# Emieeel/auto_oo

Measured on AMD Instinct MI355X. Metric: OO-VQE energy+grad evals/sec (formaldimine CAS(4e,3o)/cc-pVDZ); 2e-transform fp64 TFLOP/s vs roofline, higher is better.
Workload: dtype f64; 1 GPU; configs[1] shape: N=43 AOs, n_occ=6, CAS(4e,3o), UCCD n_theta=4, n_kappa=327; one step = one batched call evaluating energy + full gradient of all 256 geometries of the rank (256 synthetic geometries in the job, geometry g on rank g mod n_gpus); value = evaluations/s; in-order calls on one stream; geometries_per_rank=256, batched_calls=1332, calls=in order, parallelism=geometry-sharded x1, one all_gather at the end, dist_world_size=1, devices_visible=1, device_of_rank0=0

## Files before the change

### auto_oo_amd/csrc/cas.hip

```cpp
#include "plan.h"
#include "circuit_small.h"
#include <type_traits>
#include <stdlib.h>

namespace {

constexpr int HALF_WAVES = 8;
constexpr int TRI_REG_R = 3;
constexpr int tiles_depth(int zt) { return zt == 3 ? 4 : 8; }
constexpr int stream_depth(int zt) { return zt == 3 ? 2 : 3; }
constexpr int AUX_PLAIN = 0, AUX_NT = 2;

constexpr int SYM_FULL = 0, SYM_MIRROR = 1, SYM_PACKED = 2;
__device__ __forceinline__ void tri_decode(long t, int N, int& p, int& q)
{
    const double b = 2.0 * N + 1.0;
    int pp = (int)((b - sqrt(b * b - 8.0 * (double)t)) * 0.5);
    pp = pp < 0 ? 0 : (pp > N - 1 ? N - 1 : pp);
    while (pp > 0 && (long)pp * (2 * N - pp + 1) / 2 > t) --pp;
    while (pp < N - 1 && (long)(pp + 1) * (2 * N - pp) / 2 <= t) ++pp;
    p = pp;
    q = pp + (int)(t - (long)pp * (2 * N - pp + 1) / 2);
}

// ... 2354 lines not shown
            const long idx = base + u * 512 + tid;
            if (idx < (long)nrdm * n_kappa) gvec[idx] = 2.0 * (frc[u] - fcr[u]);
        }
    }
    if (fock)
        for (int idx = tid; idx < N * N; idx += 512) {
            const int m = idx / N;
            fock[idx] = m < M ? Fcol[idx] : 0.0;
        }
    if (gmat)
        for (int idx = tid; idx < N * N; idx += 512) {
            const int m = idx / N, n = idx - m * N;
            const double fmn = m < M ? Fcol[(size_t)m * N + n] : 0.0;
            const double fnm = n < M ? Fcol[(size_t)n * N + m] : 0.0;
            gmat[idx] = 2.0 * (fmn - fnm);
        }
    if (tid < nrdm) {
        const int k = tid;
        double acc = 0.0;
        for (int n = 0; n < M; ++n) acc += Epart[(size_t)k * N + n];
        if (k == 0) {
            double core = nuc;
            for (int n = 0; n < M; ++n) core += Cpart[n];
            c0[0] = core;
            E[0] = core + acc;
        } else if (dE) {
            dE[k - 1] = acc;
        }
    }
}

constexpr int TAIL_THREADS = 512;

__host__ __device__ inline bool tail_needed(int x, int y, int z, int no)
{
    const int lo = y < z ? y : z, hi = y < z ? z : y;
    if (lo >= no) return true;
    if (hi < no) return lo == hi || x == lo || x == hi;
    return x >= no || x == lo;
}
__host__ __device__ inline int tail_pitch(int NC) { return 16 * (((NC + 15) / 16) | 1); }

#ifdef OOVQE_TAIL_PROBE
constexpr int TAIL_PROBE_WGS = 512, TAIL_PROBE_MARKS = 32;
__device__ long long g_tail_probe[TAIL_PROBE_WGS][TAIL_PROBE_MARKS];
#define TAIL_MARK(i)                                                                              \
    do {                                                                                          \
        __syncthreads();                                                                          \
        if (threadIdx.x == 0 && blockIdx.x < TAIL_PROBE_WGS && (i) < TAIL_PROBE_MARKS)            \
            g_tail_probe[blockIdx.x][i] = wall_clock64();                                         \
    } while (0)
#else
#define TAIL_MARK(i) do {} while (0)
#endif

template <int KS>
__global__ __launch_bounds__(TAIL_THREADS, 2)
void cas_tail_kernel(const double* __restrict__ J, const double* __restrict__ C, const double* __restrict__ Wpre,
                     const double* __restrict__ gamma, const double* __restrict__ Gamma, int nrdm, int N, int no,
                     int na, int NC, double nuc, const double* __restrict__ nuc_arr,
                     const int32_t* __restrict__ kap_row, const int32_t* __restrict__ kap_col, int n_kappa,
                     double* __restrict__ c0, double* __restrict__ E, double* __restrict__ gvec,
                     double* __restrict__ dE, double* __restrict__ c1, double* __restrict__ c2, size_t out_stride)
{
    extern __shared__ double lds[];
    constexpr int NW = TAIL_THREADS / 64;
    constexpr int PW = (4 * KS + NW - 1) / NW;
    constexpr int GR = 2, NG = (PW + GR - 1) / GR;
    constexpr int NTN = (4 * KS + 15) / 16;
    const int M = no + na, M2 = M * M, M3 = M2 * M;
    const int na2 = na * na, na3 = na2 * na, na4 = na2 * na2;
    const int ncol = M * (M + 1) / 2, nty = (ncol + 15) / 16;
    const long tri = (long)N * (N + 1) / 2;
    const int by = blockIdx.x;
    const int tid = threadIdx.x, lane = tid & 63;
    const int wave = __builtin_amdgcn_readfirstlane(tid >> 6);
    const int lq = lane >> 4, lr = lane & 15;
    {
        const size_t gi = by;
        J += gi * nty * tri * 16;
        C += gi * (size_t)N * N;
        Wpre += gi * (size_t)N * N;
        gamma += gi * (size_t)nrdm * na2;
        Gamma += gi * (size_t)nrdm * na4;
        c0 += gi * out_stride;
        E += gi * out_stride;
        gvec += gi * out_stride;
        if (dE) dE += gi * out_stride;
        c1 += gi * out_stride;
        c2 += gi * out_stride;
        if (nuc_arr) nuc = nuc_arr[gi];
    }
    const int LDG = tail_pitch(NC), nct = (NC + 15) / 16;
    double* Gc = lds;
    double* Cl = Gc + (size_t)4 * KS * LDG;
    double* hn = Cl + (size_t)N * M;
// ... 47 lines not shown
        }
    };
    auto mfma_group = [&](const double (&af)[KS], const double (&bf)[GR][KS], const int (&tj)[4], int g) {
#pragma unroll
        for (int r = 0; r < GR; ++r) {
            const int i = g * GR + r;
            if (i >= PW) continue;
            int wv = wave;
#if defined(__HIP_DEVICE_COMPILE__)
            asm volatile("" : "+s"(wv));
#endif
            const int p = wv + NW * i;
            if (p >= 4 * KS) continue;
            d4 acc = d4{0.0, 0.0, 0.0, 0.0};
            if (p < N) {
#pragma unroll
                for (int ks = 0; ks < KS; ++ks) acc = mfma_f64(af[ks], bf[r][ks], acc);
            }
            double* row = Gc + p * LDG;
#pragma unroll
            for (int j = 0; j < 4; ++j)
                if (tj[j] >= 0) row[tj[j]] = acc[j];
        }
    };
    double bs[2][GR][KS];
    TAIL_MARK(0);
#pragma unroll
    for (int s0 = 0; s0 < 2; ++s0) load_group(bs[s0], s0 / NG, s0 % NG);

    for (int idx = tid; idx < N * M; idx += TAIL_THREADS) {
        const int q = idx / M, x = idx - q * M;
        Cl[idx] = C[(size_t)q * N + x];
    }
    for (int idx = tid; idx < N * N; idx += TAIL_THREADS) scr[idx] = Wpre[idx];
    for (int idx = tid; idx < nrdm * na2; idx += TAIL_THREADS) gml[idx] = gamma[idx];
    for (int idx = tid; idx < nrdm * na4; idx += TAIL_THREADS) Gml[idx] = Gamma[idx];
    for (int idx = tid; idx < n_kappa; idx += TAIL_THREADS) {
        krow[idx] = kap_row[idx];
        kcol[idx] = kap_col[idx];
    }
    for (int idx = tid; idx < 4 * KS * (LDG - NC); idx += TAIL_THREADS) {
        const int p = idx / (LDG - NC);
        Gc[p * LDG + NC + (idx - p * (LDG - NC))] = 0.0;
    }
    TAIL_MARK(1);
    {
        const int total = M * ncol;
        int base = 0;
        for (int i0 = 0; i0 < total; i0 += TAIL_THREADS) {
            const int i = i0 + tid;
            int x = 0, y = 0, z = 0;
            bool need = false;
            if (i < total) {
                x = i / ncol;
                tri_decode(i - x * ncol, M, y, z);
                need = tail_needed(x, y, z, no);
            }
            const unsigned long long mask = __ballot(need);
            const int below = __popcll(mask & ((1ull << lane) - 1ull));
            if (lane == 0) wcnt[wave] = __popcll(mask);
            __syncthreads();
            int pre = base, all = 0;
            for (int w = 0; w < NW; ++w) {
                const int c = wcnt[w];
                if (w < wave) pre += c;
                all += c;
            }
            if (i < total) {
                const int v = need ? pre + below : -1;
                tab[(x * M + y) * M + z] = v;
                tab[(x * M + z) * M + y] = v;
                tabp[i] = v;
            }
            __syncthreads();
            base += all;
        }
    }
    TAIL_MARK(2);
    for (int idx = tid; idx < N * M; idx += TAIL_THREADS) {
        const int n = idx / M, x = idx - n * M;
        double acc = 0.0;
        for (int q = 0; q < N; ++q) acc += scr[(size_t)n * N + q] * Cl[q * M + x];
        hn[idx] = acc;
    }
    __syncthreads();
    TAIL_MARK(3);

    {
        double af[KS];
#pragma unroll
        for (int ks = 0; ks < KS; ++ks) {
            const int q = 4 * ks + lq;
            const double c = Cl[(q < N ? q : N - 1) * M + (lr < M ? lr : 0)];
            af[ks] = (q < N && lr < M) ? c : 0.0;
        }
        auto tail_tile = [&](auto par, int ty) {
            constexpr int P = decltype(par)::value;
            const int yz = 16 * ty + lr;
            int tj[4];
#pragma unroll
            for (int j = 0; j < 4; ++j) {
                const int x = lq + 4 * j;
                tj[j] = (x < M && yz < ncol) ? tabp[x * ncol + yz] : -1;
            }
#pragma unroll
            for (int g = 0; g < NG; ++g) {
                mfma_group(af, bs[(P + g) & 1], tj, g);
                __builtin_amdgcn_sched_barrier(0);
                load_group(bs[(P + g) & 1], ty + (g + 2) / NG, (g + 2) % NG);
                __builtin_amdgcn_sched_barrier(0);
            }
        };
// ... 463 lines not shown

static size_t tail_lds_bytes(int N, int no, int na, int nrdm, int n_kappa, int* NC)
{
    const int M = no + na, M3 = M * M * M;
    Stage1Variant v;
    if (N > 48 || M > 16 || stage1_variant(N, &v)) return 0;
    int nc = 0;
    for (int x = 0; x < M; ++x)
        for (int y = 0; y < M; ++y)
            for (int z = y; z < M; ++z) nc += tail_needed(x, y, z, no) ? 1 : 0;
    *NC = nc;
    const size_t na2 = (size_t)na * na, na4 = na2 * na2;
    size_t scr = (size_t)N * N + ((size_t)M * (M * (M + 1) / 2) + 1) / 2;
    const size_t gc = (size_t)4 * tail_depth(N, v) * tail_pitch(nc);
    const size_t fe = (size_t)nrdm * M * N + (size_t)nrdm * N +
                      (size_t)N * na * na * na + (size_t)N * no * na2;
    if (fe > scr) scr = fe;
    const size_t doubles = gc + 3 * (size_t)N * M + (size_t)nrdm * (na2 + na4) + N +
                           ((size_t)M3 + TAIL_THREADS / 64 + 2 * (size_t)n_kappa + 1) / 2 + scr;
    const size_t bytes = doubles * sizeof(double);
    return bytes <= 160 * 1024 ? bytes : 0;
}

static int cas_tail_batched(const CasEvalArgs& a, const EvalPlan& p, const double* J, const double* Wpre, hipStream_t st)
{
    Stage1Variant v;
    if (int rc = stage1_variant(a.N, &v)) return rc;
#define OOVQE_LAUNCH_TAIL(KS_)                                                                    \
    do {                                                                                          \
        if (int rc_ = oovqe_ensure_dynamic_lds((const void*)cas_tail_kernel<KS_>, p.tail_lds)) return rc_; \
        hipLaunchKernelGGL((cas_tail_kernel<KS_>), dim3(a.batch), dim3(TAIL_THREADS), p.tail_lds, st, J, a.C, Wpre, \
                           a.gamma, a.Gamma, a.nrdm, a.N, a.n_occ, a.ncas, p.tail_nc, a.nuc, a.nuc_arr, a.kap_row, \
                           a.kap_col, a.n_kappa, a.out.c0, a.out.E, a.out.gvec, a.out.dE, a.out.c1, a.out.c2,       \
                           a.out_stride);                                                         \
    } while (0)
    oovqe_profile_mark_start_l(st, LABEL_P_TO_N);
    OOVQE_TAIL_DISPATCH(tail_depth(a.N, v), OOVQE_LAUNCH_TAIL)
    oovqe_profile_mark_stop(st);
#undef OOVQE_LAUNCH_TAIL
    OOVQE_CHECK_LAUNCH("cas_eval/tail");
    return 0;
}

static bool fused_plan(int N, int M, int batch, int n_cu, long chunks_opt, FusedPlan* fp)
{
    if (M > 16 || N > 48 || N < 1) return false;
    const long m2 = (long)M * M, m3 = m2 * M;
    if (chunks_opt <= 0 && (long)batch * N * N < 48L * n_cu) return false;
    long target = n_cu / batch;
    long nchunk0 = chunks_opt > 0 ? chunks_opt : target / N;
    if (nchunk0 < 1) nchunk0 = 1;
    const long cap = (2L * N * m2 - m3) / (m3 + N);
    if (cap < 1) return false;
    if (nchunk0 > cap) nchunk0 = cap;
    int qc = N, nchunk = 1;
    if (nchunk0 > 1) {
        qc = 4 * (int)((N + 4 * nchunk0 - 1) / (4 * nchunk0));
        nchunk = (N + qc - 1) / qc;
    }
    const int QR = (qc + 3) & ~3, CR = (nchunk - 1) * qc + QR;
    int ldb = (int)((m2 + 15) / 16 * 16);
    if (ldb % 32 == 0) ldb += 16;
    const size_t fixed = ((size_t)CR * 16 + 64 + 8) * sizeof(double);
    const size_t block = (size_t)QR * ldb * sizeof(double);
    const size_t task_stage = (size_t)m3 * sizeof(double);
    const long Tg = (long)nchunk * N;
    long wpg = target < 1 ? 1 : target;
// ... 290 lines not shown
                  "cas_eval: bad sizes");
    OOVQE_REQUIRE(s.batch >= 1 && s.batch <= 65535, "cas_eval: batch=%d", s.batch);
    OOVQE_REQUIRE(s.n_cu >= 1, "cas_eval: n_cu=%d", s.n_cu);
    const EvalOpts& o = s.opt;
    const int N = s.N, M = s.n_occ + s.ncas, batch = s.batch, nrdm = s.nrdm;
    const long m2 = (long)M * M, m3 = m2 * M;
    const long tri = (long)N * (N + 1) / 2;
    const long nty16 = (m2 + 15) / 16 * 16;
    const bool pq = (s.eri_flags & OOVQE_ERI_PQ_SYMMETRIC) != 0;
    p.rs = (s.eri_flags & OOVQE_ERI_RS_SYMMETRIC) != 0 && !o.sym_no_rs;

    const bool fused = !o.cas_unfused && fused_plan(N, M, batch, s.n_cu, o.fused_chunks, &p.fused);
    const bool packed = fused && pq && !o.sym_mirror && tri * nty16 + 2 * (long)N * m3 <= 2 * (long)N * N * m2;
    const bool two_step = o.sym_simple || o.sym_two_step;

    if (s.n_qubits > 0) {
        p.circuit = CIRCUIT_OWN;
        p.circuit_small = oovqe_circuit_rdms_is_small(s.n_qubits, s.ncas, nrdm, s.n_gates) != 0;
        if (p.circuit_small && o.no_ride != 1) {
            const long K = fused ? (long)p.fused.nchunk * N : N, B = fused ? m3 : (long)N * m2;
            bool ride = oovqe_small_circuit_lds_bytes(s.n_qubits, s.ncas, nrdm, s.n_gates) <= 64 * 1024 &&
                        K <= 0x7fffffffL && oovqe_contract_hosts_circuit(1, (int)K, N, B, 0, batch, o.k1);
            if (ride && fused && pq && !o.sym_mirror && o.no_ride != 2) {
                const long ntile = ((p.rs ? (long)M * (M + 1) / 2 : m2) + 15) / 16;
                if ((ntile + 1) * batch > 3L * s.n_cu) ride = false;
            }
            if (ride) p.circuit = CIRCUIT_RIDES;
        }
    }
    p.w = packed && !two_step && !o.panel_no_w && p.circuit == CIRCUIT_OWN && p.circuit_small && batch <= 32767;
    if (p.w && p.rs && s.packed && !s.t2_ready && !s.extras && 2L * batch > (long)s.n_cu && !o.tail_split)
        p.tail_lds = tail_lds_bytes(N, s.n_occ, s.ncas, nrdm, s.n_kappa, &p.tail_nc);
    if (p.tail_lds == 0 && N > m3) p.w = false;
    if (packed)
        p.path = p.tail_lds > 0 ? PATH_PACKED_TAIL : two_step ? PATH_PACKED_TWO_STEP : PATH_PACKED_SPLIT;
    else if (fused)
        p.path = PATH_FUSED;
    else
        p.path = column_fits(N, M, s.ncas) ? PATH_COLUMN : PATH_STAGED;
    OOVQE_REQUIRE(p.path != PATH_STAGED || M < N,
                  "cas_eval: the staged path needs at least one virtual orbital (N=%d M=%d)", N, M);
    if (p.path == PATH_STAGED && p.circuit == CIRCUIT_RIDES) p.circuit = CIRCUIT_OWN;

    Stage1Variant v;
    if (packed || fused)
        if (int rc = stage1_variant(N, &v)) return rc;
    if (!packed && fused) {
        p.stage1 = stage1_small(S1_FUSED, v, 0);
    } else if (!packed) {
        if (int rc = stage1_half(N, M, pq ? SYM_MIRROR : SYM_FULL, p.rs, N > 48 && s.packed, &p.stage1)) return rc;
    } else if (o.sym_simple) {
        if (int rc = stage1_half(N, M, SYM_PACKED, false, false, &p.stage1)) return rc;
    } else if (s.t2_ready && !two_step) {
        p.stage1.kernel = S1_FROM_T2;
    } else {
        p.stage1 = stage1_small(!two_step && p.rs && s.packed ? S1_TRI_REG : S1_TRI, v, two_step ? 0 : p.rs ? 2 : 1);
    }

    const size_t nb = (size_t)batch;
    size_t at = 0;
    auto block = [&](WorkBlock b, size_t doubles) { p.off[b] = at; p.len[b] = nb * doubles; at += nb * doubles; };
    if (packed) {
        block(WB_JP, (size_t)(tri * nty16));
        block(WB_T3, (size_t)N * m3);
        block(WB_GMW, (size_t)N * m3);
        if (!two_step) p.len[WB_T3] = p.w ? nb * N * N : 0;
// ... 356 lines not shown
    hipStream_t st = (hipStream_t)a.cas.stream;

    CasEvalArgs c = a.cas;
    c.gamma = a.work;
    c.Gamma = c.gamma + nb * nvec * na2;
    c.nrdm = nvec;
    c.work = a.work + nb * nvec * (na2 + na4);
    c.out = out_layout(a.out, nvec, c.n_kappa, c.ncas);
    c.out_stride = (size_t)oovqe_oo_eval_out_size(a.n_theta, c.n_kappa, c.ncas, a.derivatives);

    EvalPlan p;
    if (int rc = oovqe_eval_plan(eval_shape(c, a.n_qubits, a.n_gates), &p)) return rc;

    oovqe_circuit_job_t cj;
    if (p.circuit == CIRCUIT_RIDES) {
        cj = oovqe_circuit_job_t{.theta = a.theta, .gates = a.gates, .gamma = const_cast<double*>(c.gamma),
                                 .Gamma = const_cast<double*>(c.Gamma), .n_theta = a.n_theta, .n_gates = a.n_gates,
                                 .n_qubits = a.n_qubits, .ncas = a.cas.ncas, .n_tan = nvec - 1, .count = a.cas.batch,
                                 .init_index = a.init_index,
                                 .lds_bytes = oovqe_small_circuit_lds_bytes(a.n_qubits, a.cas.ncas, nvec, a.n_gates)};
        c.cj = &cj;
    } else {
        double *psi = nullptr, *dpsi = nullptr, *rwork = nullptr;
        if (!p.circuit_small) {
            psi = c.work + nb * oovqe_cas_eval_work_size(a.cas.N, a.cas.n_occ, a.cas.ncas, nvec);
            dpsi = psi + nb * D;
            rwork = psi + nb * nvec * D;
        }
        oovqe_profile_mark_start_l(st, LABEL_CIRCUIT);
        int rc = oovqe_circuit_rdms_w(a.theta, a.n_theta, a.gates, a.n_gates, a.n_qubits, a.cas.ncas, a.init_index,
                                      a.derivatives, a.cas.batch, psi, a.derivatives ? dpsi : nullptr,
                                      const_cast<double*>(c.gamma), const_cast<double*>(c.Gamma), rwork,
                                      p.w ? a.cas.h_ao : nullptr, p.w ? a.cas.C : nullptr, a.cas.N,
                                      p.w ? c.work + p.off[WB_T3] : nullptr, a.cas.stream);
        if (rc) return rc;
        oovqe_profile_mark_stop(st);
        if (c.rdm_event) {
            OOVQE_CHECK_HIP(hipEventRecord(c.rdm_event, st), "oo_eval: hipEventRecord");
            c.rdm_event = nullptr;
        }
    }
    return cas_eval_batched(c, p);
}

int oovqe_half_transform_batched_impl(const double* g_ao, const double* C, int N, int M, double* T2,
                                      int batch, unsigned eri_flags, oovqe_stream_t stream, double* Vk_tri)
{
    const bool pq = (eri_flags & OOVQE_ERI_PQ_SYMMETRIC) != 0;
    const bool rs = (eri_flags & OOVQE_ERI_RS_SYMMETRIC) != 0 && oovqe_opt(OOVQE_OPT_SYM_NO_RS) == 0;
    Stage1 s;
    if (int rc = stage1_half(N, M, pq ? SYM_MIRROR : SYM_FULL, rs, false, &s)) return rc;
    return half_transform_batched(g_ao, C, N, M, T2, batch, stream, s, Vk_tri);
}

extern "C" int oovqe_oo_eval_batch(const double* theta, int n_theta, const oovqe_gate_t* gates,
                                   int n_gates, int n_qubits, uint32_t init_index, const double* g_ao,
                                   const double* h_ao, const double* C, const double* nuc, int N,
                                   int n_occ, int ncas, const int32_t* kap_row, const int32_t* kap_col,
                                   int n_kappa, int derivatives, int batch, double* work, double* out,
                                   unsigned eri_flags, const double* g_packed, oovqe_stream_t stream)
{
    OOVQE_REQUIRE(nuc, "oo_eval_batch: null nuc");
    return oovqe_oo_eval_batched_impl(OoEvalArgs{
        .theta = theta, .n_theta = n_theta, .gates = gates, .n_gates = n_gates, .n_qubits = n_qubits,
        .init_index = init_index, .derivatives = derivatives, .work = work, .out = out,
        .cas = {.g_ao = g_ao, .h_ao = h_ao, .C = C, .nuc_arr = nuc, .N = N, .n_occ = n_occ, .ncas = ncas,
                .kap_row = kap_row, .kap_col = kap_col, .n_kappa = n_kappa, .batch = batch, .stream = stream,
// ... 21 lines not shown
{
    static thread_local char line[1024];
    static const char* const path_names[] = {"packed_tail", "packed_split", "packed_two_step", "fused", "column", "staged"};
    static const char* const circuit_names[] = {"none", "rides", "own"};
    static const char* const block_names[WB_COUNT] = {"Jp", "T3", "Gmw", "Cdup", "T2", "U", "Fcol", "Epart", "Cpart"};
    const EvalShape s{.N = N, .n_occ = n_occ, .ncas = ncas, .nrdm = derivatives ? 1 + n_theta : 1, .n_kappa = n_kappa,
                      .batch = batch, .eri_flags = eri_flags, .packed = have_packed != 0, .n_qubits = n_qubits,
                      .n_gates = n_gates, .n_cu = oovqe_cu_count(), .opt = oovqe_eval_opts()};
    EvalPlan p;
    if (n_qubits != 0 && n_qubits != 2 * ncas) {
        oovqe_set_error("oo_eval: n_qubits != 2*ncas");
        return nullptr;
    }
    if (oovqe_eval_plan(s, &p)) return nullptr;
    const bool k1 = p.path == PATH_PACKED_TWO_STEP || p.path == PATH_FUSED || p.path == PATH_COLUMN;
    const long M = n_occ + ncas, K = p.path == PATH_FUSED ? (long)p.fused.nchunk * N : N;
    const int hosts = k1 && oovqe_contract_hosts_circuit(1, (int)K, N, p.path == PATH_COLUMN ? N * M * M : M * M * M, 0, batch, s.opt.k1);
    size_t n = 0;
    auto add = [&](const char* fmt, auto... args) {
        if (n < sizeof(line)) n += (size_t)snprintf(line + n, sizeof(line) - n, fmt, args...);
    };
    add("path=%s; stage1=%s; circuit=%s; w=%d; launches=%ld; k1_hosts=%d; labels=", path_names[p.path], p.stage1.name,
        circuit_names[p.circuit], p.w ? 1 : 0, p.launches, hosts);
    for (int l = 0; l < LABEL_COUNT; ++l) add("%s%d", l ? "," : "", p.labels[l]);
    add("%s", "; blocks=");
    for (int b = 0, first = 1; b < WB_COUNT; ++b)
        if (p.len[b]) {
            add("%s%s@%zu+%zu", first ? "" : ",", block_names[b], p.off[b], p.len[b]);
            first = 0;
        }
    if (p.path == PATH_PACKED_TAIL) {
        Stage1Variant v;
        if (stage1_variant(N, &v)) return nullptr;
        add("; tail=cas_tail_kernel<%d>; tail_lds=%zu", tail_depth(N, v), p.tail_lds);
    }
    if (p.path == PATH_FUSED)
        add("; nchunk=%d; qc=%d; nbuf=%d; wpg=%d", p.fused.nchunk, p.fused.qc, p.fused.nbuf, p.fused.wpg);
    if (p.path == PATH_PACKED_SPLIT || p.path == PATH_PACKED_TWO_STEP || p.path == PATH_FUSED) {
        PanelGeom pg;
        const bool panel_w = p.w && p.path == PATH_PACKED_SPLIT;
        if (!oovqe_panel_geom(N, n_occ, ncas, s.nrdm, batch, panel_w, oovqe_opt(OOVQE_OPT_PANEL_ROWS), &pg)) pg = PanelGeom{};
        add("; npan=%d; npan_max=%d; rdm_chunk=%d; panel_w=%d; xcd_grid=%d", pg.npan, pg.npan_max, pg.rdm_chunk,
            panel_w ? 1 : 0, oovqe_xcd_grid(batch, oovqe_opt(OOVQE_OPT_GM_PLAIN_GRID) != 0) ? 1 : 0);
    }
    if (p.path == PATH_COLUMN) {
        ColumnGeom cg;
        if (!oovqe_column_geom(N, n_occ, ncas, s.nrdm, batch, s.n_cu, &cg)) cg = ColumnGeom{};
        add("; rdm_chunk=%d; zsplit=%d", cg.rdm_chunk, cg.zsplit);
    }
    if (p.path == PATH_STAGED) add("; staged_rows=%d", p.staged_rows ? 1 : 0);
    return line;
}

__global__ void fock_core_active_kernel(const double* __restrict__ h, const double* __restrict__ g,
                                        const double* __restrict__ gam, int N, int no, int na,
                                        double* __restrict__ FI, double* __restrict__ FA)
{
    const int idx = blockIdx.x * blockDim.x + threadIdx.x;
    if (idx >= N * N) return;
    const int m = idx / N, n = idx - m * N;
    const size_t n2 = (size_t)N * N, n3 = n2 * N;
    const double* gm = g + (size_t)m * n3;
    if (FI) {
        double acc = h[idx];
        for (int i = 0; i < no; ++i)
            acc += 2.0 * gm[(size_t)n * n2 + (size_t)i * N + i] - gm[(size_t)i * n2 + (size_t)i * N + n];
        FI[idx] = acc;
// ... 27 lines not shown
```

### auto_oo_amd/csrc/circuit.hip

```cpp
#include "internal.h"
#include <vector>
#include "circuit_small.h"

namespace {

constexpr int CIRC_THREADS = 256;
constexpr int LDS_STATE_MAX = 8192;

__device__ void apply_gate(double* st, uint32_t D, const oovqe_gate_t& g, double c, double s,
                           bool deriv)
{
    const uint32_t fm = g.mask_hi | g.mask_lo;
    const uint32_t npairs = D >> g.nfix;
    if (!deriv) {
        for (uint32_t t = threadIdx.x; t < npairs; t += CIRC_THREADS) {
            const uint32_t x = deposit(t, g) | g.mask_hi;
            const uint32_t y = x ^ fm;
            const double pi = (__popc(x & g.mask_par) & 1) ? -1.0 : 1.0;
            const double ax = st[x], ay = st[y];
            st[x] = c * ax + pi * s * ay;
            st[y] = c * ay - pi * s * ax;
        }
    } else {
        const double h = 0.5 * (double)g.sign;
// ... 292 lines not shown
        }
        const double g = reduce(part);
        if (tid == 0) gam_row[s] = g;
    }
    __syncthreads();
    const size_t set = (size_t)b * nvec + k;
    if (tid == 0) gamma[set * na2 + pq] = gam_row[q];

    const double* b0 = V0 + (size_t)(q * ncas + p) * D;
    const double* bk = Vk + (size_t)(q * ncas + p) * D;
    for (int rs = 0; rs < na2; ++rs) {
        const double* k0 = V0 + (size_t)rs * D;
        const double* kk = Vk + (size_t)rs * D;
        double part = 0.0;
        if (k == 0) {
            for (uint32_t x = tid; x < D; x += 256) part += b0[x] * k0[x];
        } else {
            for (uint32_t x = tid; x < D; x += 256) part += bk[x] * k0[x] + b0[x] * kk[x];
        }
        const double g = reduce(part);
        if (tid == 0) {
            const int r = rs / ncas, s = rs - r * ncas;
            Gamma[(set * na2 + pq) * na2 + rs] = g - (q == r ? gam_row[s] : 0.0);
        }
    }
}

__global__ __launch_bounds__(SMALL_THREADS)
void circuit_rdm_small_kernel(const double* __restrict__ theta, int n_theta,
                              const oovqe_gate_t* __restrict__ gates, int n_gates, int n_qubits,
                              int ncas, uint32_t init_index, int n_tan, double* __restrict__ psi_out,
                              double* __restrict__ dpsi_out, double* __restrict__ gamma,
                              double* __restrict__ Gamma, int batch, const double* __restrict__ h_ao,
                              const double* __restrict__ C, int N, double* __restrict__ Wpre)
{
    extern __shared__ double lds[];
    if ((int)blockIdx.x >= batch) {
        const int g = (int)blockIdx.x - batch;
        const double* __restrict__ hg = h_ao + (size_t)g * N * N;
        const double* __restrict__ Cg = C + (size_t)g * N * N;
        double* __restrict__ Wg = Wpre + (size_t)g * N * N;
        double* hs = lds;
        double* cs = lds + (size_t)N * N;
        constexpr int IT = (48 * 48 + SMALL_THREADS - 1) / SMALL_THREADS;
        double rh[IT], rc[IT];
#pragma unroll
        for (int it = 0; it < IT; ++it) {
            const int idx = threadIdx.x + it * SMALL_THREADS;
            const int ic = idx < N * N ? idx : 0;
            rh[it] = hg[ic];
            rc[it] = Cg[ic];
        }
#pragma unroll
        for (int it = 0; it < IT; ++it) {
            const int idx = threadIdx.x + it * SMALL_THREADS;
            if (idx < N * N) { hs[idx] = rh[it]; cs[idx] = rc[it]; }
        }
        __syncthreads();
        for (int idx = threadIdx.x; idx < N * N; idx += SMALL_THREADS) {
            const int n = idx / N, q = idx - n * N;
            double a0 = 0.0, a1 = 0.0;
            int p = 0;
            for (; p + 1 < N; p += 2) {
                a0 += cs[p * N + n] * hs[p * N + q];
                a1 += cs[(p + 1) * N + n] * hs[(p + 1) * N + q];
            }
            if (p < N) a0 += cs[p * N + n] * hs[p * N + q];
            Wg[idx] = a0 + a1;
        }
        return;
    }
    circuit_rdm_small_body(theta, n_theta, gates, n_gates, n_qubits, ncas, init_index, n_tan, psi_out,
                           dpsi_out, gamma, Gamma, (int)blockIdx.x, lds);
}

__device__ void apply_gate_mode(double* st, uint32_t D, const oovqe_gate_t& g, double c, double s,
                                int mode)
{
    const uint32_t fm = g.mask_hi | g.mask_lo;
    const uint32_t npairs = D >> g.nfix;
    const double h = 0.5 * (double)g.sign;
    for (uint32_t t = threadIdx.x; t < npairs; t += CIRC_THREADS) {
        const uint32_t x = deposit(t, g) | g.mask_hi;
        const uint32_t y = x ^ fm;
        const double pi = (__popc(x & g.mask_par) & 1) ? -1.0 : 1.0;
        const double ax = st[x], ay = st[y];
        const double nx = c * ax + pi * s * ay, ny = c * ay - pi * s * ax;
        if (mode == 0) {
            st[x] = nx;
            st[y] = ny;
        } else if (mode == 1) {
            st[x] = h * (-s * ax + pi * c * ay);
            st[y] = h * (-s * ay - pi * c * ax);
        } else {
            st[x] = -0.25 * nx;
            st[y] = -0.25 * ny;
        }
    }
    if (mode != 0) {
        for (uint32_t x = threadIdx.x; x < D; x += CIRC_THREADS) {
            const uint32_t f = x & fm;
// ... 195 lines not shown
    OOVQE_REQUIRE(n_tan == 0 || dpsi, "rdms_tangent: dpsi required when n_tan > 0");
    OOVQE_REQUIRE(n_qubits == 2 * ncas && ncas >= 1 && ncas <= 13 && batch >= 1 && n_tan >= 0,
                  "rdms_tangent: bad sizes n_qubits=%d ncas=%d", n_qubits, ncas);
    const uint32_t D = 1u << n_qubits;
    const int na2 = ncas * ncas;
    const int nvec = 1 + n_tan;
    OOVQE_REQUIRE(batch <= 65535 && (long)nvec * na2 <= 65535, "rdms_tangent: grid too large");
    hipStream_t st = (hipStream_t)stream;
    hipLaunchKernelGGL(epq_apply_multi_kernel, dim3((D + 255) / 256, nvec * na2, batch), dim3(256),
                       0, st, psi, dpsi, n_qubits, ncas, nvec, work);
    OOVQE_CHECK_LAUNCH("rdms_tangent/epq_apply");
    hipLaunchKernelGGL(rdm_tangent_gram_kernel, dim3(na2, nvec, batch), dim3(256), 0, st, psi, dpsi,
                       work, n_qubits, ncas, nvec, gamma, Gamma);
    OOVQE_CHECK_LAUNCH("rdms_tangent/gram");
    return 0;
}

static size_t small_lds_bytes(int n_qubits, int ncas, int nvec, int n_gates)
{
    return oovqe_small_circuit_lds_bytes(n_qubits, ncas, nvec, n_gates);
}

extern "C" int oovqe_circuit_rdms_is_small(int n_qubits, int ncas, int nvec, int n_gates)
{
    return n_qubits <= 10 && small_lds_bytes(n_qubits, ncas, nvec, n_gates) <= 150 * 1024;
}

extern "C" int oovqe_circuit_rdms(const double* theta, int n_theta, const oovqe_gate_t* gates,
                                  int n_gates, int n_qubits, int ncas, uint32_t init_index,
                                  int want_tangents, int batch, double* psi, double* dpsi,
                                  double* gamma, double* Gamma, double* work, oovqe_stream_t stream)
{
    return oovqe_circuit_rdms_w(theta, n_theta, gates, n_gates, n_qubits, ncas, init_index, want_tangents, batch, psi,
                                dpsi, gamma, Gamma, work, nullptr, nullptr, 0, nullptr, stream);
}

int oovqe_circuit_rdms_w(const double* theta, int n_theta, const oovqe_gate_t* gates, int n_gates, int n_qubits,
                         int ncas, uint32_t init_index, int want_tangents, int batch, double* psi, double* dpsi,
                         double* gamma, double* Gamma, double* work, const double* h_ao, const double* C, int N,
                         double* Wpre, oovqe_stream_t stream)
{
    OOVQE_REQUIRE(theta && gates && gamma && Gamma, "circuit_rdms: null pointer");
    OOVQE_REQUIRE(n_qubits == 2 * ncas && ncas >= 1 && ncas <= 13, "circuit_rdms: bad sizes");
    OOVQE_REQUIRE(n_theta >= 1 && n_gates >= 1 && batch >= 1, "circuit_rdms: bad sizes");
    const int n_tan = want_tangents ? n_theta : 0;
    const int nvec = 1 + n_tan;
    size_t lds_bytes = small_lds_bytes(n_qubits, ncas, nvec, n_gates);
    OOVQE_REQUIRE(!Wpre || (h_ao && C && N >= 1 && N <= 48 && oovqe_circuit_rdms_is_small(n_qubits, ncas, nvec, n_gates) &&
                            batch <= 32767),
                  "circuit_rdms: W = C^T h rides with the one-workgroup circuit kernel (N <= 48)");
    if (Wpre && (size_t)2 * N * N * sizeof(double) > lds_bytes) lds_bytes = (size_t)2 * N * N * sizeof(double);
    if (oovqe_circuit_rdms_is_small(n_qubits, ncas, nvec, n_gates)) {
        if (int rc_lds = oovqe_ensure_dynamic_lds((const void*)circuit_rdm_small_kernel, 150 * 1024)) return rc_lds;
        hipLaunchKernelGGL(circuit_rdm_small_kernel, dim3(Wpre ? 2 * batch : batch), dim3(SMALL_THREADS), lds_bytes,
                           (hipStream_t)stream, theta, n_theta, gates, n_gates, n_qubits, ncas,
                           init_index, n_tan, psi, dpsi, gamma, Gamma, batch, h_ao, C, N, Wpre);
        OOVQE_CHECK_LAUNCH("circuit_rdms/small");
        return 0;
    }
    OOVQE_REQUIRE(psi && work && (!want_tangents || dpsi),
                  "circuit_rdms: psi/dpsi/work buffers required for this size");
    int rc = circuit_state_launch(theta, n_theta, gates, n_gates, n_qubits, init_index, batch, psi,
                                  want_tangents ? dpsi : nullptr, want_tangents ? work : nullptr, stream);
    if (rc) return rc;
    return oovqe_rdms_tangent(psi, want_tangents ? dpsi : nullptr, n_qubits, ncas, n_tan, batch,
                              gamma, Gamma, work, stream);
}

extern "C" int oovqe_circuit_second_tangents(const double* theta, int n_theta,
                                             const oovqe_gate_t* gates, int n_gates, int n_qubits,
                                             uint32_t init_index, const int32_t* pairs, int n_pairs,
                                             double* out, double* scratch, oovqe_stream_t stream)
{
    OOVQE_REQUIRE(theta && gates && pairs && out && scratch, "second_tangents: null pointer");
    OOVQE_REQUIRE(n_qubits >= 2 && n_qubits <= 26 && n_pairs >= 1 && n_gates >= 1 && n_theta >= 1,
                  "second_tangents: bad sizes");
    hipLaunchKernelGGL(circuit_second_tangent_kernel, dim3(n_pairs), dim3(CIRC_THREADS), 0,
                       (hipStream_t)stream, theta, n_theta, gates, n_gates, n_qubits, init_index, pairs, out,
                       scratch);
    OOVQE_CHECK_LAUNCH("second_tangents");
    return 0;
}

extern "C" int oovqe_circuit_hessian_assemble(const double* gamma, const double* Gamma,
                                              const double* c1, const double* c2, int ncas,
                                              const int32_t* pairs, int n_pairs, int n_theta,
                                              double* H, oovqe_stream_t stream)
{
    OOVQE_REQUIRE(gamma && Gamma && c1 && c2 && pairs && H, "circuit_hessian: null pointer");
// ... 86 lines not shown
```

### auto_oo_amd/csrc/internal.h

```cpp
#pragma once
#include "common.h"

int oovqe_mode_contract_impl(const double* T, const double* Cm, double* out, long A, int K, int J,
                             long B, int ldc, int last, hipStream_t st);
int oovqe_mode_contract_batched(const double* T, const double* Cm, double* out, long A, int K, int J,
                                long B, int ldc, int last, int batch, long t_bs, long c_bs, long o_bs,
                                hipStream_t st, const oovqe_circuit_job_t* cj = nullptr);
struct ContractOpts {
    int force_nt;
    bool force_wide, no_pair;
};
ContractOpts oovqe_contract_opts();
int oovqe_contract_hosts_circuit(long A, int K, int J, long B, int last, int batch, const ContractOpts& o);

int oovqe_contract_pair_ok(const double* T, const double* out, long A, long B, int nt, int ngroups, int batch,
                           long t_bs, long o_bs);
int oovqe_contract_pair_grid(long A, long B, int ngroups, int batch, long* n_items, long* grid_x);
int oovqe_contract_pair_launch(const double* T, const double* Cm, double* out, long A, int K, int J, long B,
                               int ldc, int nt, int ngroups, int deep, int batch, long t_bs, long c_bs,
                               long o_bs, hipStream_t st);

int oovqe_circuit_rdms_w(const double* theta, int n_theta, const oovqe_gate_t* gates, int n_gates, int n_qubits,
                         int ncas, uint32_t init_index, int want_tangents, int batch, double* psi, double* dpsi,
                         double* gamma, double* Gamma, double* work, const double* h_ao, const double* C, int N,
                         double* Wpre, oovqe_stream_t stream);
int oovqe_circuit_hessian_batched_impl(const double* theta, int n_theta, const oovqe_gate_t* gates,
                                       int n_gates, int n_qubits, int ncas, uint32_t init_index,
                                       const double* c1, const double* c2, long c1_bs, long c2_bs,
                                       const int32_t* pairs, int n_pairs, int batch, double* work, double* H,
                                       long ldh, long h_bs, oovqe_stream_t stream);

struct OutSlab {
    double *c0, *E, *dE, *gvec, *c1, *c2;
};
inline OutSlab out_layout(double* out, int nvec, int n_kappa, int ncas)
{
    OutSlab o;
    o.c0 = out;
    o.E = out + 1;
    o.dE = out + 2;
    o.gvec = o.dE + (nvec > 1 ? nvec - 1 : 1);
    o.c1 = o.gvec + (size_t)nvec * n_kappa;
    o.c2 = o.c1 + (size_t)ncas * ncas;
    return o;
}

struct CasEvalArgs {
    const double *g_ao, *h_ao, *C;
    const double *gamma, *Gamma;
    int nrdm;
    double nuc;
    const double* nuc_arr;
    int N, n_occ, ncas;
    const int32_t *kap_row, *kap_col;
    int n_kappa;
    double* work;
    OutSlab out;
    size_t out_stride;
// ... 32 lines not shown
```

### auto_oo_amd/csrc/plan.h

```cpp
#pragma once
#include "internal.h"

enum EvalPath {
    PATH_PACKED_TAIL = 0,
    PATH_PACKED_SPLIT,
    PATH_PACKED_TWO_STEP,
    PATH_FUSED,
    PATH_COLUMN,
    PATH_STAGED
};
enum CircuitPlace {
    CIRCUIT_NONE = 0,
    CIRCUIT_RIDES,
    CIRCUIT_OWN
};
enum Stage1Kernel {
    S1_HALF, S1_STREAM, S1_TILES,
    S1_FUSED,
    S1_TRI, S1_TRI_REG,
    S1_FROM_T2
};
enum { LABEL_STAGE1 = 0, LABEL_CIRCUIT, LABEL_P_TO_N, LABEL_COLUMN, LABEL_FINAL, LABEL_Q_TO_X, LABEL_COUNT };
enum WorkBlock { WB_JP = 0, WB_T3, WB_GMW, WB_CDUP, WB_T2, WB_U, WB_FCOL, WB_EPART, WB_CPART, WB_COUNT };

// ... 14 lines not shown
struct FusedPlan {
    int nchunk, qc, nbuf, ldb, wpg;
    size_t lds_bytes;
};

struct EvalOpts {
    int fused_chunks, no_ride;
    bool cas_unfused, sym_no_rs, sym_mirror, sym_simple, sym_two_step, panel_no_w, tail_split;
    ContractOpts k1;
};
EvalOpts oovqe_eval_opts();

struct EvalShape {
    int N, n_occ, ncas, nrdm, n_kappa, batch;
    unsigned eri_flags;
    bool packed;
    bool t2_ready;
    bool extras;
    int n_qubits, n_gates;
    int n_cu;
    EvalOpts opt;
};

struct EvalPlan {
    EvalPath path;
    Stage1 stage1;
    FusedPlan fused;
    CircuitPlace circuit;
    bool circuit_small;
    bool w;
    bool rs;
    int tail_nc;
    size_t tail_lds;
    bool staged_rows;
    size_t off[WB_COUNT], len[WB_COUNT];
    int labels[LABEL_COUNT];
    long launches;
};

int oovqe_eval_plan(const EvalShape& s, EvalPlan* plan);

struct PanelGeom {
    int npan, npan_max, rdm_chunk;
    size_t lds_bytes;
};
struct ColumnGeom {
    int rdm_chunk, zsplit;
    size_t lds_bytes;
};
bool oovqe_panel_geom(int N, int n_occ, int ncas, int nrdm, int batch, bool w, int panel_rows, PanelGeom* g);
bool oovqe_column_geom(int N, int n_occ, int ncas, int nrdm, int batch, int n_cu, ColumnGeom* g);
inline bool oovqe_xcd_grid(int batch, bool plain_grid) { return batch > 1 && !plain_grid; }
```

Before: 608,000 evals/s.

## Precompute h_mo and tail lookup tables in the circuit kernel's W side-blocks

The extra workgroups that ride alongside the small circuit kernel now also build the tail's compaction tables and finish the second half-transform (W·C giving h_mo). They store these in the Wpre slot instead of the full N×N W matrix. The tail kernel then only copies them into LDS, skipping its ballot/prefix-scan table build and the N·M·N h_mo loop, which shortens its serial prologue. The W=C^T h product is also register-blocked over four q columns. This costs extra LDS for the side-blocks and adds more work to the circuit kernel's side path.

```diff
diff --git a/auto_oo_amd/csrc/cas.hip b/auto_oo_amd/csrc/cas.hip
--- a/auto_oo_amd/csrc/cas.hip
+++ b/auto_oo_amd/csrc/cas.hip
@@ -2410,13 +2410,6 @@
 
 constexpr int TAIL_THREADS = 512;
 
-__host__ __device__ inline bool tail_needed(int x, int y, int z, int no)
-{
-    const int lo = y < z ? y : z, hi = y < z ? z : y;
-    if (lo >= no) return true;
-    if (hi < no) return lo == hi || x == lo || x == hi;
-    return x >= no || x == lo;
-}
 __host__ __device__ inline int tail_pitch(int NC) { return 16 * (((NC + 15) / 16) | 1); }
 
 #ifdef OOVQE_TAIL_PROBE
@@ -2439,7 +2432,7 @@
                      int na, int NC, double nuc, const double* __restrict__ nuc_arr,
                      const int32_t* __restrict__ kap_row, const int32_t* __restrict__ kap_col, int n_kappa,
                      double* __restrict__ c0, double* __restrict__ E, double* __restrict__ gvec,
-                     double* __restrict__ dE, double* __restrict__ c1, double* __restrict__ c2, size_t out_stride)
+                     double* __restrict__ dE, double* __restrict__ c1, double* __restrict__ c2, size_t out_stride, int pre)
 {
     extern __shared__ double lds[];
     constexpr int NW = TAIL_THREADS / 64;
@@ -2553,7 +2546,14 @@
         const int q = idx / M, x = idx - q * M;
         Cl[idx] = C[(size_t)q * N + x];
     }
-    for (int idx = tid; idx < N * N; idx += TAIL_THREADS) scr[idx] = Wpre[idx];
+    if (pre) {
+        const int* tabs = reinterpret_cast<const int*>(Wpre + (size_t)N * M);
+        for (int idx = tid; idx < N * M; idx += TAIL_THREADS) hn[idx] = Wpre[idx];
+        for (int idx = tid; idx < M3; idx += TAIL_THREADS) tab[idx] = tabs[idx];
+        for (int idx = tid; idx < M * ncol; idx += TAIL_THREADS) tabp[idx] = tabs[M3 + idx];
+    } else {
+        for (int idx = tid; idx < N * N; idx += TAIL_THREADS) scr[idx] = Wpre[idx];
+    }
     for (int idx = tid; idx < nrdm * na2; idx += TAIL_THREADS) gml[idx] = gamma[idx];
     for (int idx = tid; idx < nrdm * na4; idx += TAIL_THREADS) Gml[idx] = Gamma[idx];
     for (int idx = tid; idx < n_kappa; idx += TAIL_THREADS) {
@@ -2565,7 +2565,7 @@
         Gc[p * LDG + NC + (idx - p * (LDG - NC))] = 0.0;
     }
     TAIL_MARK(1);
-    {
+    if (!pre) {
         const int total = M * ncol;
         int base = 0;
         for (int i0 = 0; i0 < total; i0 += TAIL_THREADS) {
@@ -2598,7 +2598,7 @@
         }
     }
     TAIL_MARK(2);
-    for (int idx = tid; idx < N * M; idx += TAIL_THREADS) {
+    for (int idx = tid; idx < (pre ? 0 : N * M); idx += TAIL_THREADS) {
         const int n = idx / M, x = idx - n * M;
         double acc = 0.0;
         for (int q = 0; q < N; ++q) acc += scr[(size_t)n * N + q] * Cl[q * M + x];
@@ -3128,7 +3128,7 @@
         hipLaunchKernelGGL((cas_tail_kernel<KS_>), dim3(a.batch), dim3(TAIL_THREADS), p.tail_lds, st, J, a.C, Wpre, \
                            a.gamma, a.Gamma, a.nrdm, a.N, a.n_occ, a.ncas, p.tail_nc, a.nuc, a.nuc_arr, a.kap_row, \
                            a.kap_col, a.n_kappa, a.out.c0, a.out.E, a.out.gvec, a.out.dE, a.out.c1, a.out.c2,       \
-                           a.out_stride);                                                         \
+                           a.out_stride, p.tail_pre ? 1 : 0);                                     \
     } while (0)
     oovqe_profile_mark_start_l(st, LABEL_P_TO_N);
     OOVQE_TAIL_DISPATCH(tail_depth(a.N, v), OOVQE_LAUNCH_TAIL)
@@ -3485,6 +3485,7 @@
     if (p.w && p.rs && s.packed && !s.t2_ready && !s.extras && 2L * batch > (long)s.n_cu && !o.tail_split)
         p.tail_lds = tail_lds_bytes(N, s.n_occ, s.ncas, nrdm, s.n_kappa, &p.tail_nc);
     if (p.tail_lds == 0 && N > m3) p.w = false;
+    p.tail_pre = p.tail_lds > 0 && oovqe_tail_inputs_doubles(N, M) <= (long)N * N;
     if (packed)
         p.path = p.tail_lds > 0 ? PATH_PACKED_TAIL : two_step ? PATH_PACKED_TWO_STEP : PATH_PACKED_SPLIT;
     else if (fused)
@@ -3907,7 +3908,8 @@
                                       a.derivatives, a.cas.batch, psi, a.derivatives ? dpsi : nullptr,
                                       const_cast<double*>(c.gamma), const_cast<double*>(c.Gamma), rwork,
                                       p.w ? a.cas.h_ao : nullptr, p.w ? a.cas.C : nullptr, a.cas.N,
-                                      p.w ? c.work + p.off[WB_T3] : nullptr, a.cas.stream);
+                                      p.w ? c.work + p.off[WB_T3] : nullptr,
+                                      p.tail_pre ? a.cas.n_occ + a.cas.ncas : 0, a.cas.n_occ, a.cas.stream);
         if (rc) return rc;
         oovqe_profile_mark_stop(st);
         if (c.rdm_event) {
@@ -3995,7 +3997,7 @@
     if (p.path == PATH_PACKED_TAIL) {
         Stage1Variant v;
         if (stage1_variant(N, &v)) return nullptr;
-        add("; tail=cas_tail_kernel<%d>; tail_lds=%zu", tail_depth(N, v), p.tail_lds);
+        add("; tail=cas_tail_kernel<%d>; tail_lds=%zu; tail_pre=%d", tail_depth(N, v), p.tail_lds, p.tail_pre ? 1 : 0);
     }
     if (p.path == PATH_FUSED)
         add("; nchunk=%d; qc=%d; nbuf=%d; wpg=%d", p.fused.nchunk, p.fused.qc, p.fused.nbuf, p.fused.wpg);
diff --git a/auto_oo_amd/csrc/circuit.hip b/auto_oo_amd/csrc/circuit.hip
--- a/auto_oo_amd/csrc/circuit.hip
+++ b/auto_oo_amd/csrc/circuit.hip
@@ -348,7 +348,7 @@
                               int ncas, uint32_t init_index, int n_tan, double* __restrict__ psi_out,
                               double* __restrict__ dpsi_out, double* __restrict__ gamma,
                               double* __restrict__ Gamma, int batch, const double* __restrict__ h_ao,
-                              const double* __restrict__ C, int N, double* __restrict__ Wpre)
+                              const double* __restrict__ C, int N, double* __restrict__ Wpre, int tail_m, int tail_no)
 {
     extern __shared__ double lds[];
     if ((int)blockIdx.x >= batch) {
@@ -358,6 +358,7 @@
         double* __restrict__ Wg = Wpre + (size_t)g * N * N;
         double* hs = lds;
         double* cs = lds + (size_t)N * N;
+        double* ws = cs + (size_t)N * N;
         constexpr int IT = (48 * 48 + SMALL_THREADS - 1) / SMALL_THREADS;
         double rh[IT], rc[IT];
 #pragma unroll
@@ -367,22 +368,87 @@
             rh[it] = hg[ic];
             rc[it] = Cg[ic];
         }
+        if (tail_m) {
+            const int M = tail_m, ncol = M * (M + 1) / 2;
+            int* tab = reinterpret_cast<int*>(Wg + (size_t)N * M);
+            int* tabp = tab + M * M * M;
+            int* wcnt = reinterpret_cast<int*>(lds);
+            constexpr int NW = SMALL_THREADS / 64;
+            const int lane = threadIdx.x & 63, wave = threadIdx.x >> 6;
+            const int total = M * ncol;
+            int base = 0;
+            for (int i0 = 0; i0 < total; i0 += SMALL_THREADS) {
+                const int i = i0 + threadIdx.x;
+                int x = 0, y = 0, z = 0;
+                bool need = false;
+                if (i < total) {
+                    x = i / ncol;
+                    z = i - x * ncol;
+                    while (z >= M - y) { z -= M - y; ++y; }
+                    z += y;
+                    need = tail_needed(x, y, z, tail_no);
+                }
+                const unsigned long long mask = __ballot(need);
+                const int below = __popcll(mask & ((1ull << lane) - 1ull));
+                if (lane == 0) wcnt[wave] = __popcll(mask);
+                __syncthreads();
+                int pre = base, all = 0;
+                for (int w = 0; w < NW; ++w) {
+                    const int c = wcnt[w];
+                    if (w < wave) pre += c;
+                    all += c;
+                }
+                if (i < total) {
+                    const int v = need ? pre + below : -1;
+                    tab[(x * M + y) * M + z] = v;
+                    tab[(x * M + z) * M + y] = v;
+                    tabp[i] = v;
+                }
+                __syncthreads();
+                base += all;
+            }
+        }
 #pragma unroll
         for (int it = 0; it < IT; ++it) {
             const int idx = threadIdx.x + it * SMALL_THREADS;
             if (idx < N * N) { hs[idx] = rh[it]; cs[idx] = rc[it]; }
         }
         __syncthreads();
-        for (int idx = threadIdx.x; idx < N * N; idx += SMALL_THREADS) {
-            const int n = idx / N, q = idx - n * N;
-            double a0 = 0.0, a1 = 0.0;
+        const int QG = (N + 3) / 4;
+        double* wout = tail_m ? ws : Wg;
+        for (int item = threadIdx.x; item < N * QG; item += SMALL_THREADS) {
+            const int n = item / QG, qq = item - n * QG;
+            int qj[4];
+#pragma unroll
+            for (int j = 0; j < 4; ++j) qj[j] = qq + j * QG < N ? qq + j * QG : qq;
+            double a0[4] = {0.0, 0.0, 0.0, 0.0}, a1[4] = {0.0, 0.0, 0.0, 0.0};
             int p = 0;
             for (; p + 1 < N; p += 2) {
-                a0 += cs[p * N + n] * hs[p * N + q];
-                a1 += cs[(p + 1) * N + n] * hs[(p + 1) * N + q];
+                const double c0 = cs[p * N + n], c1 = cs[(p + 1) * N + n];
+#pragma unroll
+                for (int j = 0; j < 4; ++j) {
+                    a0[j] += c0 * hs[p * N + qj[j]];
+                    a1[j] += c1 * hs[(p + 1) * N + qj[j]];
+                }
             }
-            if (p < N) a0 += cs[p * N + n] * hs[p * N + q];
-            Wg[idx] = a0 + a1;
+            if (p < N) {
+                const double c0 = cs[p * N + n];
+#pragma unroll
+                for (int j = 0; j < 4; ++j) a0[j] += c0 * hs[p * N + qj[j]];
+            }
+#pragma unroll
+            for (int j = 0; j < 4; ++j)
+                if (qq + j * QG < N) wout[n * N + qq + j * QG] = a0[j] + a1[j];
+        }
+        if (tail_m) {
+            __syncthreads();
+            const int M = tail_m;
+            for (int idx = threadIdx.x; idx < N * M; idx += SMALL_THREADS) {
+                const int n = idx / M, x = idx - n * M;
+                double acc = 0.0;
+                for (int q = 0; q < N; ++q) acc += ws[(size_t)n * N + q] * cs[q * N + x];
+                Wg[idx] = acc;
+            }
         }
         return;
     }
@@ -644,13 +710,13 @@
                                   double* gamma, double* Gamma, double* work, oovqe_stream_t stream)
 {
     return oovqe_circuit_rdms_w(theta, n_theta, gates, n_gates, n_qubits, ncas, init_index, want_tangents, batch, psi,
-                                dpsi, gamma, Gamma, work, nullptr, nullptr, 0, nullptr, stream);
+                                dpsi, gamma, Gamma, work, nullptr, nullptr, 0, nullptr, 0, 0, stream);
 }
 
 int oovqe_circuit_rdms_w(const double* theta, int n_theta, const oovqe_gate_t* gates, int n_gates, int n_qubits,
                          int ncas, uint32_t init_index, int want_tangents, int batch, double* psi, double* dpsi,
                          double* gamma, double* Gamma, double* work, const double* h_ao, const double* C, int N,
-                         double* Wpre, oovqe_stream_t stream)
+                         double* Wpre, int tail_m, int tail_no, oovqe_stream_t stream)
 {
     OOVQE_REQUIRE(theta && gates && gamma && Gamma, "circuit_rdms: null pointer");
     OOVQE_REQUIRE(n_qubits == 2 * ncas && ncas >= 1 && ncas <= 13, "circuit_rdms: bad sizes");
@@ -661,12 +727,16 @@
     OOVQE_REQUIRE(!Wpre || (h_ao && C && N >= 1 && N <= 48 && oovqe_circuit_rdms_is_small(n_qubits, ncas, nvec, n_gates) &&
                             batch <= 32767),
                   "circuit_rdms: W = C^T h rides with the one-workgroup circuit kernel (N <= 48)");
-    if (Wpre && (size_t)2 * N * N * sizeof(double) > lds_bytes) lds_bytes = (size_t)2 * N * N * sizeof(double);
+    OOVQE_REQUIRE(tail_m == 0 || (Wpre && tail_m >= 1 && tail_m <= N && tail_no >= 0 && tail_no <= tail_m &&
+                                  oovqe_tail_inputs_doubles(N, tail_m) <= (long)N * N),
+                  "circuit_rdms: h_mo and the tail's tables (M=%d) do not fit the slot of W (N=%d)", tail_m, N);
+    const size_t w_bytes = (size_t)(tail_m ? 3 : 2) * N * N * sizeof(double);
+    if (Wpre && w_bytes > lds_bytes) lds_bytes = w_bytes;
     if (oovqe_circuit_rdms_is_small(n_qubits, ncas, nvec, n_gates)) {
         if (int rc_lds = oovqe_ensure_dynamic_lds((const void*)circuit_rdm_small_kernel, 150 * 1024)) return rc_lds;
         hipLaunchKernelGGL(circuit_rdm_small_kernel, dim3(Wpre ? 2 * batch : batch), dim3(SMALL_THREADS), lds_bytes,
                            (hipStream_t)stream, theta, n_theta, gates, n_gates, n_qubits, ncas,
-                           init_index, n_tan, psi, dpsi, gamma, Gamma, batch, h_ao, C, N, Wpre);
+                           init_index, n_tan, psi, dpsi, gamma, Gamma, batch, h_ao, C, N, Wpre, tail_m, tail_no);
         OOVQE_CHECK_LAUNCH("circuit_rdms/small");
         return 0;
     }
diff --git a/auto_oo_amd/csrc/internal.h b/auto_oo_amd/csrc/internal.h
--- a/auto_oo_amd/csrc/internal.h
+++ b/auto_oo_amd/csrc/internal.h
@@ -23,7 +23,19 @@
 int oovqe_circuit_rdms_w(const double* theta, int n_theta, const oovqe_gate_t* gates, int n_gates, int n_qubits,
                          int ncas, uint32_t init_index, int want_tangents, int batch, double* psi, double* dpsi,
                          double* gamma, double* Gamma, double* work, const double* h_ao, const double* C, int N,
-                         double* Wpre, oovqe_stream_t stream);
+                         double* Wpre, int tail_m, int tail_no, oovqe_stream_t stream);
+
+__host__ __device__ inline bool tail_needed(int x, int y, int z, int no)
+{
+    const int lo = y < z ? y : z, hi = y < z ? z : y;
+    if (lo >= no) return true;
+    if (hi < no) return lo == hi || x == lo || x == hi;
+    return x >= no || x == lo;
+}
+inline long oovqe_tail_inputs_doubles(int N, int M)
+{
+    return (long)N * M + ((long)M * M * M + (long)M * (M * (M + 1) / 2) + 1) / 2;
+}
 int oovqe_circuit_hessian_batched_impl(const double* theta, int n_theta, const oovqe_gate_t* gates,
                                        int n_gates, int n_qubits, int ncas, uint32_t init_index,
                                        const double* c1, const double* c2, long c1_bs, long c2_bs,
diff --git a/auto_oo_amd/csrc/plan.h b/auto_oo_amd/csrc/plan.h
--- a/auto_oo_amd/csrc/plan.h
+++ b/auto_oo_amd/csrc/plan.h
@@ -70,6 +70,7 @@
     bool rs;
     int tail_nc;
     size_t tail_lds;
+    bool tail_pre;
     bool staged_rows;
     size_t off[WB_COUNT], len[WB_COUNT];
     int labels[LABEL_COUNT];
```

Result: slower. 599,400 evals/s (-1.4%).
